# ltiao/bore

Measured on AMD Instinct MI355X. Metric: BO-iterations/sec (fit+argmax), 16-16-1 MLP, higher is better.
Workload: dtype f32; 1 GPU; BASELINE config 4 (= config 1 x independent loops): Branin-2D, 16-16-1 MLP, q=0.25, 200 epochs, batch 64, 3 L-BFGS-B restarts from 1024 samples; loops_per_gpu=512, total_loops=512, schedule=async, N_start=15, N_end=217, parallelism=replica-shard x1

## Files before the change

bore_amd/csrc/bore_argmax.hip:

```cpp
#include <hip/hip_runtime.h>

#include <cmath>
#include <cstdlib>
#include <cstring>

#include "host_common.h"
#include "lbfgsb.h"
#include "mlp_device.h"
#include "mlp_regs.h"
#include "mlp_point.h"
#include "arg_bf16_mfma.h"

using namespace bore;

__device__ __forceinline__ void labels_body(const double *y, int N, double vi, float *z,
                                            double *tau_out, const int *ids, const int *its,
                                            int n_init, long long cap, double gamma,
                                            long long model, int it_now = -1) {
  extern __shared__ float smem[];
  double *ys = reinterpret_cast<double *>(smem);
  long long stride = N;
  if (ids) {
    N = n_init + (it_now >= 0 ? it_now : uniform_i32(its[model]));
    model = uniform_i64(ids[model]);
// ... 293 lines not shown
__global__ __launch_bounds__(BORE_THREADS) void screen_topk_kernel(const ScreenArgs a) {
  screen_body<SHAPE, BF16, MODE>(a, blockIdx.x);
}

struct SampleSpec {
  uint64_t seed;
  int64_t model_index0, draw_index;
  const double *low, *high;
};

struct ScreenRequest {
  const bore_mlp_desc *desc; int n_models; const float *theta; const double *X_init; const SampleSpec *spec;
  int64_t n_samples; int x_shared, num_starts; double *x0; int32_t *idx; float *pred;
};

struct AcqKnobs { long long coop_grid = 1LL << 22, queue = -1; int waves = -1, big = -1, occ2 = -1, screen_split = -1; };
static AcqKnobs acq_knobs() {
  auto env = [](const char *name, long long unset) { return getenv(name) ? atoll(getenv(name)) : unset; };
  return AcqKnobs{env("BORE_LBFGSB_COOP_GRID", 1LL << 22), env("BORE_LBFGSB_QUEUE", -1), (int)env("BORE_LBFGSB_WAVES", -1),
                  (int)env("BORE_LBFGSB_BIG", -1), (int)env("BORE_LBFGSB_OCC2", -1), (int)env("BORE_SCREEN_SPLIT", -1)};
}

struct ScreenPlan {
  ScreenArgs a;
  size_t lds_floats;
  int flavour, parts;
};

static int screen_plan(const bore_mlp_desc *desc, int n_models, int64_t n_samples, int num_starts, bool pred,
                       const AcqKnobs &knobs, int cus, bool batch, ScreenPlan &p) {
  ScreenArgs &a = p.a;
  if (n_samples < 1 || n_samples > (1 << 20)) return fail(BORE_E_INVALID, "screen_topk: n_samples out of range");
  if (num_starts < 1 || num_starts > n_samples) return fail(BORE_E_INVALID, "screen_topk: need 1 <= num_starts <= n_samples");
  int n_pad = 1;
  while (n_pad < n_samples) n_pad <<= 1;
// ... 129 lines not shown
  (void)hipMemcpyToSymbol(HIP_SYMBOL(lbfgsb::g_lb_pp), zz, sizeof(zz));
  return (int)hipMemcpyToSymbol(HIP_SYMBOL(lbfgsb::g_lb_phase), z, sizeof(z));
}
extern "C" int bore_debug_lpp(unsigned long long *out) {
  return (int)hipMemcpyFromSymbol(out, HIP_SYMBOL(lbfgsb::g_lb_pp),
                                  sizeof(unsigned long long) * LB_PP_MAX * 64);
}
#define BORE_LCLOCK() clock64()
#else
#define BORE_LCLOCK() 0LL
#endif

#define BORE_POINT_SHAPE(S) ((S) != 1)


template <int SHAPE, bool BF16 = false, bool LEAN = false, bool ALWAYS_COOP = false, bool MAYQ = true, int PUBLISH = 0>
__device__ __forceinline__ void lbfgsb_body(const LbfgsbArgs &a, const long long model,
                                            const int block_y, const int it_now = -1) {
  extern __shared__ float smem[];
  constexpr MlpLayout Lc = bore_static_layout(SHAPE > 0 ? SHAPE : 0, 2, BORE_BATCH_MAX);
  const long long c_enter = BORE_LCLOCK();
  const MlpLayout &L = begin_kernel<SHAPE>(Lc, a.L, smem, a.total, a.o_layout);
  const long long c_begun = BORE_LCLOCK();
  int tid = threadIdx.x;
  BORE_OPAQUE_TID(tid);
  const int wv = __builtin_amdgcn_readfirstlane(tid >> 6), lane = tid & 63;
  const long long lid = a.ids ? uniform_i64(a.ids[model]) : model;
  const int n_lay = layer_count<SHAPE>(L), D = (bore_shape_takes_fewer_inputs(SHAPE) && !BF16) ? a.d_in : L.w[0];
  const int p0 = block_y * a.PB;
  const int np = min(a.PB, a.R - p0);
  float *th = smem, *tile = smem + a.o_tile, *vals = smem + a.o_vals;
  double *blo = reinterpret_cast<double *>(smem + a.o_box), *bhi = blo + D;
  int *bnbd = reinterpret_cast<int *>(bhi + D);
// ... 24 lines not shown
    while (__hip_atomic_exchange(a.big_locks + sl, 1, __ATOMIC_ACQUIRE, __HIP_MEMORY_SCOPE_AGENT) != 0)
      sl = sl + 1 == BORE_BIG_SLOTS ? 0 : sl + 1;
    qnext[1] = sl;
    qnext[2] = 0;
  }
  const int myrow = coop ? wv * 16 : wv * 16 + lane;
  const lbfgsb::Coop cp = (ALWAYS_COOP || coop) ? lbfgsb::Coop{lane, 64} : lbfgsb::Coop{0, 1};
  __syncthreads();
  double *my_big = nullptr;
  int big_slot = 0;
  if (use_big) {
    big_slot = uniform_i32(qnext[1]);
    my_big = a.big + ((size_t)big_slot * 8 + wv) * (size_t)a.big_wave;
  }
  const long long c_staged = BORE_LCLOCK();
  if (wv >= np) {
    if (use_big && lane == 0 && atomicAdd(qnext + 2, 1) == NW - 1)
      __hip_atomic_store(a.big_locks + big_slot, 0, __ATOMIC_RELEASE, __HIP_MEMORY_SCOPE_AGENT);
    return;
  }
  double *res = reinterpret_cast<double *>(smem + a.o_res);
  int *cnt = reinterpret_cast<int *>(res + (multi ? np : 4) * (D + 3));
  for (int pass = 0; pass < passes; ++pass) {
  int myp;
  if (queue) {
    int nxt = wv;
    if (pass > 0) {
      if (lane == 0) nxt = atomicAdd(qnext, 1);
      nxt = __builtin_amdgcn_readfirstlane(nxt);
    }
    myp = nxt < np ? nxt : -1;
  } else {
    myp = coop ? (wv + 4 * pass < np ? wv + 4 * pass : -1)
               : ((lane < 16 && lane * 4 + wv < np) ? lane * 4 + wv : -1);
// ... 130 lines not shown
          if constexpr (LEAN) {
            net.load_fwd(thw);
            net.template load_bwd<Net::n, 1>(thw);
          }
          static_assert(Net::KC0 == 1, "two inputs: one k-chunk");
          float xin[Net::KC0];
          xin[0] = q4 == 0 ? (float)x0 : (q4 == 1 ? (float)x1 : 0.f);
          __builtin_amdgcn_sched_barrier(0);
          const float Tv = net.fg(thw, xin, a.transform, a.sign);
          s.f = (double)__uint_as_float(__builtin_amdgcn_readfirstlane(__float_as_uint(Tv)));
          g0 = (double)__uint_as_float(__builtin_amdgcn_readfirstlane(__float_as_uint(net.d[0][0][0])));
          g1 = (double)__uint_as_float(__builtin_amdgcn_readfirstlane(__float_as_uint(net.d[0][0][1])));
          t_fg += BORE_LCLOCK() - c1;
          ++n_rounds;
        };
        lbfgsb::lbfgsb_advance<SHAPE != 1>(st, wk, blo, bhi, bnbd, a.opt, cp, evaluate, evaluate2);
      } else {
        lbfgsb::lbfgsb_advance<SHAPE != 1>(st, wk, blo, bhi, bnbd, a.opt, cp, evaluate);
      }
      t_adv = BORE_LCLOCK() - c0 - t_fg;
      done = true;
    }
  }
  if constexpr (ALWAYS_COOP) {
  } else {
  for (int round = 0; !direct && round < a.max_rounds; ++round) {
    int pending = 0;
    const long long c0 = BORE_LCLOCK();
    if (!done) {
      const int rc = lbfgsb::lbfgsb_advance<SHAPE != 1>(st, wk, blo, bhi, bnbd, a.opt, cp);
      if (rc == lbfgsb::LB_NEED_FG) {
// ... 156 lines not shown
    for (int d = 0; d < D; ++d) put(d, best >= 0 ? res[best * (D + 3) + 3 + d] : 0.0);
    put(D, (double)best);
    put(D + 1, nfev_sum);
    put(D + 2, nfev_max);
    if (a.stamps) {
      const long long *s = a.stamps + lid * 4;
      const long long now = wall_clock64();
      put(D + 3, (double)(s[1] - s[0]));
      put(D + 4, (double)(s[2] - s[1]));
      put(D + 5, (double)(s[3] - s[2]));
      put(D + 6, (double)(now - s[3]));
    } else {
      for (int i = 3; i < 7; ++i) put(D + i, 0.0);
    }
    put(D + 7, exec_sum);
    if constexpr (PUBLISH == 1) {
      asm volatile("s_waitcnt vmcnt(0)" ::: "memory");
      if (a.flag_by_store) {
        __threadfence_system();
        __hip_atomic_store(a.flag + lid, it_done + 1, __ATOMIC_RELEASE, __HIP_MEMORY_SCOPE_SYSTEM);
      } else {
        (void)__hip_atomic_exchange(a.flag + lid, it_done + 1, __ATOMIC_RELAXED, __HIP_MEMORY_SCOPE_SYSTEM);
      }
    } else {
      __threadfence_system();
      __hip_atomic_store(a.flag + lid, it_done + 1, __ATOMIC_RELEASE, __HIP_MEMORY_SCOPE_SYSTEM);
    }
  }
  }
  if (use_big) {
    asm volatile("s_waitcnt vmcnt(0)" ::: "memory");
    if (lane == 0 && atomicAdd(qnext + 2, 1) == NW - 1)
      __hip_atomic_store(a.big_locks + big_slot, 0, __ATOMIC_RELEASE, __HIP_MEMORY_SCOPE_AGENT);
  }
}

template <int SHAPE, bool BF16 = false>
__global__ __launch_bounds__(BORE_THREADS) void lbfgsb_kernel(const LbfgsbArgs a) {
  lbfgsb_body<SHAPE, BF16>(a, blockIdx.x, blockIdx.y);
}

template <int SHAPE, bool BF16 = false>
__global__ __launch_bounds__(BORE_THREADS, 2) void lbfgsb_kernel_occ2(const LbfgsbArgs a) {
// ... 399 lines not shown
```

bore_amd/csrc/bore_engine.hip:

```cpp
#include <hip/hip_runtime.h>

#include <chrono>
#include <cmath>
#include <cstdint>
#include <cstdlib>
#include <cstring>
#include <atomic>
#include <initializer_list>
#include <mutex>
#include <new>
#include <thread>
#include <vector>

#include <sched.h>

#include "../../include/bore_hip.h"
#include "host_common.h"
#include "mlp_shapes.h"

namespace {

struct Mt19937 {
  uint32_t key[624];
  int pos;
// ... 354 lines not shown
int async_create(bore_engine *e, const double *X0, const double *y0) {
  const size_t L = e->cfg.n_loops, D = e->D, R = e->cfg.num_starts, n0 = e->cfg.n_init;
  if (R > 16) return fail(BORE_E_UNSUPPORTED, "engine_create: async_loops needs num_starts <= 16");
  e->as = new (std::nothrow) Async();
  if (!e->as) return fail(BORE_E_HIP, "engine_create: out of memory");
  Async &A = *e->as;
  int rc;
  if ((rc = async_alloc(e, n0 * 2 > 128 ? n0 * 2 : 128))) return rc;
  {
    const bore_engine_cfg &c = e->cfg;
    IterEngine &E = A.eng;
    E.desc = &e->desc; E.theta = e->theta; E.adam_m = e->adam_m; E.adam_v = e->adam_v; E.adam_t = e->adam_t;
    E.gamma = c.gamma; E.epochs = c.epochs; E.batch_size = c.batch_size; E.seed = c.seed; E.loop_id0 = c.loop_id0;
    E.adam = &c.adam; E.num_samples = c.num_samples; E.low = e->low.data(); E.high = e->high.data();
    E.num_starts = c.num_starts; E.transform = c.transform; E.opts = &c.lbfgsb; E.n_loops = c.n_loops;
  }
  std::vector<float> x32(L * n0 * D);
  for (size_t i = 0; i < x32.size(); ++i) x32[i] = (float)X0[i];
  HIP_TRY(hipMemcpy2D(A.eng.X_seen, A.cap * D * 8, X0, n0 * D * 8, n0 * D * 8, L, hipMemcpyHostToDevice));
  HIP_TRY(hipMemcpy2D(A.eng.y_seen, A.cap * 8, y0, n0 * 8, n0 * 8, L, hipMemcpyHostToDevice));
  HIP_TRY(hipMemcpy2D(A.eng.X32, A.cap * D * 4, x32.data(), n0 * D * 4, n0 * D * 4, L, hipMemcpyHostToDevice));
  if ((rc = pin_alloc(&A.result, L * (D + 8))) || (rc = pin_alloc(&A.flag, L)) ||
      (rc = dev_alloc(&A.stamps, L * 4)))
    return rc;
  std::memset(A.flag, 0, L * 4);
  HIP_TRY(hipMemset(A.stamps, 0, L * 4 * 8));
  {
    int dev = 0, khz = 0;
    HIP_TRY(hipGetDevice(&dev));
    if (hipDeviceGetAttribute(&khz, hipDeviceAttributeWallClockRate, dev) == hipSuccess && khz > 0)
// ... 766 lines not shown
```

bore_amd/csrc/bore_iter.hip:

```cpp

struct QueueEntry {
  int lid, it;
};

struct IterArgs {
  FitArgs f;
  ScreenArgs s;
  LbfgsbArgs b;
  double *X_seen, *y_seen;
  float *X32, *z;
  const double *x_new, *y_new;
  long long *stamps;
  double gamma;
  int D;
  const int *targets;
  const double *ynew;
  const int *yseq;
  int *parked;
  const int *abort_flag;
  long long wait_ticks;
  const QueueEntry *q_ring;
  unsigned long long *q_head;
  int q_mask;
  const unsigned long long *q_tail_host;
// ... 3 lines not shown
__device__ __forceinline__ double load_host_f64(const double *p) {
  const long long v = __hip_atomic_load(reinterpret_cast<const long long *>(p), __ATOMIC_RELAXED,
                                        __HIP_MEMORY_SCOPE_SYSTEM);
  return __longlong_as_double(v);
}

#define BORE_LAG_YIELD_Q 3
__device__ __forceinline__ void phase_handoff() {
  __builtin_amdgcn_fence(__ATOMIC_RELEASE, "workgroup");
  asm volatile("s_waitcnt vmcnt(0) lgkmcnt(0)" ::: "memory");
  __syncthreads();
  __builtin_amdgcn_fence(__ATOMIC_ACQUIRE, "workgroup");
  asm volatile("buffer_inv sc0\n\ts_waitcnt vmcnt(0)" ::: "memory");
}

template <int SHAPE, bool LOCAL = false>
__device__ __forceinline__ void iteration_once(const IterArgs *__restrict__ pa,
                                                         const long long slot, const int it,
                                                         const bool staged, const long long t_begin = 0) {
  const IterArgs &a = *pa;
  const long long lid = uniform_i64(a.f.ids[slot]), cap = a.f.cap;
  long long *stp = a.stamps ? a.stamps + lid * 4 : nullptr;
  if (stp && threadIdx.x == 0) stp[0] = t_begin ? t_begin : wall_clock64();
  if (it > 0) {
    const long long row = a.f.n_init + it - 1;
    for (int d = threadIdx.x; d < a.D; d += blockDim.x) {
      const double v = staged ? a.x_new[slot * a.D + d] : load_host_f64(a.ynew + lid * (a.D + 1) + d);
      a.X_seen[(lid * cap + row) * a.D + d] = v;
      a.X32[(lid * cap + row) * a.D + d] = (float)v;
    }
    if (threadIdx.x == 0)
// ... 13 lines not shown
  }
  fit_body<SHAPE>(a.f, slot, it);
  if (stp && threadIdx.x == 0) stp[2] = wall_clock64();
  if constexpr (LOCAL) phase_handoff();
  else {
    __threadfence();
    __syncthreads();
  }
  screen_body<SHAPE, false>(a.s, slot, it);
  if (stp && threadIdx.x == 0) stp[3] = wall_clock64();
  if constexpr (LOCAL) phase_handoff();
  else {
    __threadfence();
    __syncthreads();
  }
  lbfgsb_body<SHAPE, false, true, true, false, LOCAL ? 1 : 0>(a.b, slot, 0, it);
}

template <int SHAPE, bool RESIDENT, int OCC = 2>
__global__ __launch_bounds__(BORE_THREADS, OCC) void iteration_kernel(const IterArgs *__restrict__ pa) {
  const long long slot = blockIdx.x;
  const int it_first = uniform_i32(pa->f.its[slot]);
  if constexpr (!RESIDENT) {
    typedef const __attribute__((address_space(4))) IterArgs *IterArgsConst1;
    const IterArgs &a = *(const IterArgs *)(IterArgsConst1) reinterpret_cast<unsigned long long>(pa);
    const long long lid = uniform_i64(a.f.ids[slot]), cap = a.f.cap;
    const int it = it_first;
    long long *stp = a.stamps ? a.stamps + lid * 4 : nullptr;
    if (stp && threadIdx.x == 0) stp[0] = wall_clock64();
    if (it > 0) {
      const long long row = a.f.n_init + it - 1;
      for (int d = threadIdx.x; d < a.D; d += blockDim.x) {
        const double v = a.x_new[slot * a.D + d];
        a.X_seen[(lid * cap + row) * a.D + d] = v;
// ... 3 lines not shown
    }
    __threadfence();
    __syncthreads();
    labels_body(a.y_seen, 0, 0.0, a.z, nullptr, a.f.ids, a.f.its, a.f.n_init, cap, a.gamma, slot);
    if (stp && threadIdx.x == 0) stp[1] = wall_clock64();
    __threadfence();
    __syncthreads();
    fit_body<SHAPE>(a.f, slot);
    if (stp && threadIdx.x == 0) stp[2] = wall_clock64();
    __threadfence();
    __syncthreads();
    screen_body<SHAPE, false>(a.s, slot);
    if (stp && threadIdx.x == 0) stp[3] = wall_clock64();
    __threadfence();
    __syncthreads();
    lbfgsb_body<SHAPE, false, true, true, false>(a.b, slot, 0);
    if (a.targets && threadIdx.x == 0 && it + 1 < a.targets[slot])
      __hip_atomic_store(a.parked + lid, it + 1, __ATOMIC_RELEASE, __HIP_MEMORY_SCOPE_SYSTEM);
    return;
  }
  __shared__ __attribute__((aligned(16))) int s_go4[4];
  const int target = pa->targets ? uniform_i32(pa->targets[slot]) : it_first + 1;
  int *prog;
  {
    unsigned long long pb = reinterpret_cast<unsigned long long>(pa) + offsetof(IterArgs, progress);
    asm volatile("" : "+s"(pb));
    prog = reinterpret_cast<int *>(pb);
  }
  for (int it = it_first;;) {
    {
      const int total = __hip_atomic_load(prog, __ATOMIC_RELAXED, __HIP_MEMORY_SCOPE_AGENT);
      const int n_wg = (int)gridDim.x;
      const int lead = uniform_i32((it - it_first) * n_wg - total);
      if (lead < -(n_wg >> 1)) __builtin_amdgcn_s_setprio(3);
      else if (lead > (n_wg >> 1)) __builtin_amdgcn_s_setprio(0);
      else __builtin_amdgcn_s_setprio(1);
    }
    unsigned long long pa_bits = reinterpret_cast<unsigned long long>(pa);
    asm volatile("" : "+s"(pa_bits));
    typedef const __attribute__((address_space(4))) IterArgs *IterArgsConst;
    iteration_once<SHAPE, true>((const IterArgs *)(IterArgsConst)pa_bits, slot, it, it == it_first);
    __syncthreads();
    ++it;
    if (threadIdx.x == 0) __hip_atomic_fetch_add(prog, 1, __ATOMIC_RELAXED, __HIP_MEMORY_SCOPE_AGENT);
    if (it >= target) break;
    if (threadIdx.x == 0) {
      const long long lid = pa->f.ids[slot], wait_ticks = pa->wait_ticks;
      const int *yseq = pa->yseq + lid, *abort_flag = pa->abort_flag;
      int go = 0;
      const long long t0 = wall_clock64();
      for (;;) {
        if (__hip_atomic_load(yseq, __ATOMIC_RELAXED, __HIP_MEMORY_SCOPE_SYSTEM) >= it) {
          asm volatile("" ::: "memory");
          go = 1;
          break;
        }
// ... 14 lines not shown
      s_go4[0] = go;
    }
    __syncthreads();
    const int go = uniform_i32(s_go4[0]);
    __syncthreads();
    if (!go) break;
  }
}

#ifdef BORE_QUEUE_STAMP_DRAW
__device__ long long g_wg_start[4096][2];
extern "C" int bore_debug_wg_starts(long long *out) {
  return (int)hipMemcpyFromSymbol(out, HIP_SYMBOL(g_wg_start), sizeof(long long) * 4096 * 2);
}
#endif
template <int SHAPE, int OCC = 2>
__global__ __launch_bounds__(BORE_THREADS, OCC) void queue_kernel(const IterArgs *__restrict__ pa) {
  __shared__ __attribute__((aligned(16))) int s_q4[4];
#ifdef BORE_QUEUE_STAMP_DRAW
  if (threadIdx.x == 0 && blockIdx.x < 4096) {
    g_wg_start[blockIdx.x][0] = wall_clock64();
    const unsigned hw = __builtin_amdgcn_s_getreg((4) | (0 << 6) | (31 << 11));
    const unsigned xcc = __builtin_amdgcn_s_getreg((20) | (0 << 6) | (31 << 11));
    g_wg_start[blockIdx.x][1] = ((long long)xcc << 32) | hw;
  }
#endif
  for (;;) {
    if (threadIdx.x == 0) {
#ifdef BORE_QUEUE_STAMP_DRAW
      const long long t_draw = wall_clock64();
      s_q4[2] = (int)(t_draw & 0xffffffffll);
// ... 33 lines not shown
      s_q4[0] = lid;
      s_q4[1] = it;
    }
    __syncthreads();
    const int lid = uniform_i32(s_q4[0]), it = uniform_i32(s_q4[1]);
#ifdef BORE_QUEUE_STAMP_DRAW
    const long long t_begin = ((long long)s_q4[3] << 32) | (unsigned)s_q4[2];
#else
    const long long t_begin = 0;
#endif
    __syncthreads();
    if (lid < 0) break;
    unsigned long long pa_bits = reinterpret_cast<unsigned long long>(pa);
    asm volatile("" : "+s"(pa_bits));
    typedef const __attribute__((address_space(4))) IterArgs *IterArgsConst;
    iteration_once<SHAPE>((const IterArgs *)(IterArgsConst)pa_bits, (long long)lid, it, false, t_begin);
    __syncthreads();
  }
}

static int iteration_shape(const bore_mlp_desc *desc) {
  if (desc->compute != BORE_COMPUTE_F32) return 0;
  const int f = bore_kernel_flavour(desc, true);
  if (f == 1) return 1;
  if (f == 5 && desc->input_dim == 16 && bore_flavour_on(5)) return 5;
  return 0;
}

static constexpr bool fused_flavour_on(int shape) { return shape == 1 || bore_flavour_on(shape); }
static constexpr int fused_most_per_cu(int shape) { return shape == 5 ? 2 : 3; }

// ... 28 lines not shown
  const bore_mlp_desc *desc;
  float *theta, *adam_m, *adam_v;
  int64_t *adam_t;
  double *X_seen, *y_seen;
  float *X32, *z;
  double gamma;
  int epochs, batch_size;
  uint64_t seed;
  int64_t loop_id0;
  const bore_adam_cfg *adam;
  int64_t num_samples;
  const double *low, *high;
  int num_starts, transform;
  const bore_lbfgsb_opts *opts;
  int n_loops;
};

struct Worker {
  hipStream_t stream = nullptr;
  hipEvent_t done = nullptr, ev[4] = {nullptr, nullptr, nullptr, nullptr};
  bool busy = false;
  int32_t *h_int = nullptr, *d_int = nullptr;
  double *h_dbl = nullptr, *d_dbl = nullptr;
  double *x0 = nullptr, *x = nullptr, *jac = nullptr, *fun = nullptr;
  int32_t *idx = nullptr, *info = nullptr;
  IterArgs *h_args = nullptr, *d_args = nullptr;
  size_t stage_bytes = 0;
};

struct IterQueue {
  const QueueEntry *ring;
  unsigned long long *head;
  int mask;
  const unsigned long long *tail_host;
  int wgs;
};

struct IterPlan {
  int shape;
  size_t lds_bytes;
  size_t part_bytes[4];
};

static int iteration_plan(const IterEngine &E, const Worker &w, int n_slots, IterArgs *h, IterPlan *plan) {
  if (!g_batch) return fail(BORE_E_INVALID, "iteration_launch: no batch set");
  const int64_t cap = g_batch->cap;
  FitPlan fit;
  ScreenPlan screen;
  LbfgsbPlan restarts;
  int rc = fit_build(FitRequest{E.desc, n_slots, E.theta, E.adam_m, E.adam_v, E.adam_t, E.X32, E.z, cap, E.epochs,
                                E.batch_size, nullptr, E.seed, E.loop_id0, 0, E.adam, nullptr},
                     fit);
  if (rc) return rc < 0 ? rc : fail(BORE_E_INVALID, "iteration_launch: epochs must be positive");
  h->f = fit.a;
  const size_t lf = fit.lds_floats;
  const int sf = fit.flavour;
// ... 15 lines not shown
  h->targets = g_batch->targets;
  h->ynew = g_batch->ynew; h->yseq = g_batch->yseq; h->parked = g_batch->parked;
  h->abort_flag = g_batch->abort_flag;
  const bool resident = g_batch->targets && g_batch->ynew && g_batch->yseq && g_batch->parked &&
                        g_batch->abort_flag;
  if (!resident) h->targets = nullptr;
  h->wait_ticks = resident ? g_batch->wait_ticks : 0;
  h->gamma = E.gamma;
  h->D = E.desc->input_dim;
  h->progress = 0;
  h->q_ring = nullptr; h->q_head = nullptr; h->q_mask = 0; h->q_tail_host = nullptr;
  size_t floats = lf > ls ? lf : ls;
  floats = floats > lb ? floats : lb;
  const size_t labels_floats = 2 * ((size_t)cap + 2);
  floats = floats > labels_floats ? floats : labels_floats;
  *plan = IterPlan{shape, floats * 4, {lf * 4, ls * 4, lb * 4, labels_floats * 4}};
  return bore_with_flavour<fused_flavour_on>(FusedFlavours{}, shape, [&](auto S) {
    int rc = 0;
    if ((rc = allow_lds(iteration_kernel<S(), true, 2>, floats * 4)) || (rc = allow_lds(iteration_kernel<S(), false, 2>, floats * 4)) ||
        (rc = allow_lds(queue_kernel<S(), 2>, floats * 4)))
      return rc;
    if constexpr (fused_most_per_cu(S()) == 3)
      if ((rc = allow_lds(iteration_kernel<S(), true, 3>, floats * 4)) || (rc = allow_lds(queue_kernel<S(), 3>, floats * 4))) return rc;
    return 0;
  });
}

template <typename K>
static int fused_launch(K kernel, int workgroups, const IterPlan &p, const Worker &w) {
  hipLaunchKernelGGL(kernel, dim3(workgroups), dim3(BORE_THREADS), p.lds_bytes, w.stream, (const IterArgs *)w.d_args);
  HIP_TRY(hipGetLastError());
  return 0;
}

static int iteration_launch_queue(const IterEngine &E, Worker &w, int n_slots, const IterQueue &q) {
  IterArgs *h = w.h_args;
  IterPlan p;
  if (const int rc = iteration_plan(E, w, n_slots, h, &p)) return rc;
  if (q.wgs < 1 || !q.ring || !q.head || !q.tail_host || !g_batch->ynew || !g_batch->abort_flag)
    return fail(BORE_E_INVALID, "iteration_launch: incomplete work queue");
  h->q_ring = q.ring; h->q_head = q.head; h->q_mask = q.mask; h->q_tail_host = q.tail_host;
  h->targets = nullptr;
  h->wait_ticks = 0;
  HIP_TRY(hipMemcpyAsync(w.d_args, h, sizeof(IterArgs), hipMemcpyHostToDevice, w.stream));
  return bore_with_flavour<fused_flavour_on>(FusedFlavours{}, p.shape, [&](auto S) {
    if constexpr (fused_most_per_cu(S()) == 3)
      if (q.wgs > 2 * device_cus()) return fused_launch(queue_kernel<S(), 3>, q.wgs, p, w);
    return fused_launch(queue_kernel<S(), 2>, q.wgs, p, w);
  });
}

static int iteration_launch(const IterEngine &E, Worker &w, int n_slots) {
  IterArgs *h = w.h_args;
  IterPlan p;
  int rc;
  if ((rc = iteration_plan(E, w, n_slots, h, &p))) return rc;
  if (h->wait_ticks > 0) {
    int per_cu = 0;
    if ((rc = iteration_loops_per_cu(p.shape, p.lds_bytes, &per_cu))) return rc;
    if (getenv("BORE_ASYNC_DEBUG"))
      fprintf(stderr, "[bore] fused kernel: %zu B of LDS per loop (fit %zu, screen %zu, restarts %zu, labels %zu), %d loops per CU\n",
              p.lds_bytes, p.part_bytes[0], p.part_bytes[1], p.part_bytes[2], p.part_bytes[3], per_cu);
    if (g_batch->resident_loops > per_cu * device_cus()) h->wait_ticks = 0;
  }
  HIP_TRY(hipMemcpyAsync(w.d_args, h, w.stage_bytes, hipMemcpyHostToDevice, w.stream));
  return bore_with_flavour<fused_flavour_on>(FusedFlavours{}, p.shape, [&](auto S) {
    if constexpr (fused_most_per_cu(S()) == 3)
      if (h->wait_ticks > 0 && g_batch->resident_loops > 2 * device_cus()) return fused_launch(iteration_kernel<S(), true, 3>, n_slots, p, w);
    if (h->wait_ticks > 0) return fused_launch(iteration_kernel<S(), true, 2>, n_slots, p, w);
    return fused_launch(iteration_kernel<S(), false, 2>, n_slots, p, w);
  });
}
```

bore_amd/csrc/lbfgsb.h:

```cpp
#pragma once
#include <math.h>
#include <stdint.h>

#include <type_traits>

#if defined(__HIPCC__)
#define LB_HD __host__ __device__ __forceinline__
#define LB_HDN __host__ __device__ __forceinline__
#else
#define LB_HD inline
#define LB_HDN
#endif

namespace lbfgsb {

enum { LB_NEED_FG = 1, LB_DONE = 2 };

enum {
  T_START = 0, T_NEW_X = 1, T_FG = 3, T_CONVERGENCE = 4, T_STOP = 5, T_ERROR = 7, T_ABNORMAL = 8
};
enum {
  M_NONE = 0, M_PGTOL = 401, M_FACTR = 402, M_MAXFUN = 502, M_MAXITER = 504,
  M_NO_FEASIBLE = 701, M_FACTR_NEG = 702, M_M_LE_0 = 711, M_N_LE_0 = 712, M_INVALID_NBD = 713
};
// ... 1567 lines not shown
    if (nbd[i] == 2 || nbd[i] == 3) xi = fmin(xi, u[i]);
    w.x[i] = xi;
    w.g[i] = 0.0;
  }
  s.f = 0.0;
  s.stage = S_INIT;
  s.task = T_START;
  s.msg = M_NONE;
  s.nit = 0;
  s.nfev = 0;
  s.status = 2;
}

struct ReverseCommunication {};
struct NoTwoVariableForm {};
template <bool VL = true, class FG = ReverseCommunication, class FG2 = NoTwoVariableForm>
LB_HD int lbfgsb_advance(State &s, const Work &w, const double *l, const double *u,
                         const int *nbd, const Options &opt, const Coop coop_in = Coop{0, 1},
                         FG fg = FG{}, FG2 fg2 = FG2{}) {
  constexpr bool DIRECT = !std::is_same<FG, ReverseCommunication>::value;
  constexpr bool TWO = DIRECT && !std::is_same<FG2, NoTwoVariableForm>::value;
  Coop coop = coop_in;
  const int n = LB_UNI(s.n, coop_in), m = LB_UNI(s.m, coop_in);
  bool first_ls = false;
  bool resume_ls = (s.stage == S_FG_LNSRCH);

  if (s.stage == S_FINISHED) return LB_DONE;
  bool big_stale = w.vm == LB_BIG_LAZY;
  if (!DIRECT && big_stale && s.stage == S_INIT) zero_big(w, m, coop_in);
  LB_MARK(s, 15);

  auto save_evaluated_point = [&]() {
    LB_PHASE_BEGIN(20);
    for (int i = coop.lane; i < n; i += coop.nl) { w.xlast[i] = w.x[i]; w.glast[i] = w.g[i]; }
    LB_LANES_SYNC();
    s.flast = s.f;
// ... 112 lines not shown
      s.ginit = s.gtest = s.gx = s.gy = s.finit = s.fx = s.fy = s.stx = s.sty = s.stmin = s.stmax = 0.0;
      s.width = s.width1 = 0.0;
      s.xstep = s.gd = s.gdold = s.stp = s.dtd = s.dnorm = s.stpmx = s.fold = 0.0;
      s.ifun = s.iback = 0;
      s.iword = -1;
      if (!s.cnstnd && s.col > 0) {
        LB_EVENT(s, EV_UNCONSTRAINED_ITERATION);
        for (int i = coop.lane; i < n; i += coop.nl) w.z[i] = w.x[i];
        LB_LANES_SYNC();
        s.wrk = s.updatd;
        s.nseg = 0;
      } else {
        const IterArgs ia{n, m, LB_UNI(s.col, coop), LB_UNI(s.head, coop), LB_UNI(s.nfree, coop),
                          LB_UNI(s.nenter, coop), LB_UNI(s.ileave, coop), LB_UNI(s.updatd, coop),
                          LB_UNI(s.iupdat, coop), s.theta, s.sbgnrm, coop};
        LB_PHASE_BEGIN(21);
        const int rc = cauchy<VL>(ia, w, l, u, nbd);
        LB_PHASE_END(0);
        s.nseg = rc >> 8;
        if (rc & 0xff) {
          LB_EVENT(s, EV_CAUCHY_SINGULAR_REFRESH);
          refresh_memory(s);
          continue;
        }
        {
          LB_PHASE_BEGIN(22);
          freev<VL>(s, w, coop);
          LB_PHASE_END(8);
        }
        if (s.nenter > 0) LB_EVENT(s, EV_ENTER);
        if (s.ileave < n + 1) LB_EVENT(s, EV_LEAVE);
        s.nact = n - s.nfree;
      }
      if (s.nfree == 0) LB_EVENT(s, EV_NFREE_ZERO);
      if (s.nfree != 0 && s.col != 0) {
        const IterArgs ia{n, m, LB_UNI(s.col, coop), LB_UNI(s.head, coop), LB_UNI(s.nfree, coop),
                          LB_UNI(s.nenter, coop), LB_UNI(s.ileave, coop), LB_UNI(s.updatd, coop),
                          LB_UNI(s.iupdat, coop), s.theta, s.sbgnrm, coop};
        if (s.wrk) {
          LB_PHASE_BEGIN(23);
          if (DIRECT && big_stale) {
            zero_big(w, m, coop);
            big_stale = false;
          }
          const int fk = formk(ia, w);
          LB_PHASE_END(1);
          if (fk) { LB_EVENT(s, EV_FORMK_REFRESH); refresh_memory(s); continue; }
        }
        int rc;
        {
          LB_PHASE_BEGIN(24);
          const int cm = cmprlb(s, w, coop);
          LB_PHASE_END(2);
          if (cm) { LB_EVENT(s, EV_CMPRLB_REFRESH); refresh_memory(s); continue; }
        }
        {
          LB_PHASE_BEGIN(25);
          rc = subsm<VL>(ia, w, l, u, nbd);
          LB_PHASE_END(3);
        }
        s.iword = rc >> 8;
        if (rc & 0xff) { LB_EVENT(s, EV_SUBSM_REFRESH); refresh_memory(s); continue; }
        if (s.iword == 1) LB_EVENT(s, EV_SUBSM_HIT_BOUND);
      }
      {
        LB_PHASE_BEGIN(26);
        for (int i = coop.lane; i < n; i += coop.nl) w.d[i] = w.z[i] - w.x[i];
        LB_LANES_SYNC();
        LB_PHASE_END(12);
      }
      first_ls = true;
    }

    s.info = 0;
    int ls_rc;
    {
      LB_PHASE_BEGIN(27);
      ls_rc = lnsrlb<VL>(s, w, l, u, nbd, first_ls ? 1 : 0, coop);
// ... 183 lines not shown
```

Baseline: 291,000 BO-iterations/s.

## Offload L-BFGS-B formk to idle helper waves via an LDS job board

Adds a workgroup-local job board so that waves left idle (when there are 4 or fewer restarts per block) can compute formk for active restarts. The restart wave posts its formk job and runs cmprlb meanwhile. It also posts a speculative formk before the Cauchy step, double-buffering the big matrix so the speculative result can be committed if no variables enter or leave. This aims to hide formk latency on the critical path, at the cost of atomic handshakes, spin-waiting, extra LDS for the spare buffers, and extra kernel instantiations. It is enabled by default for shape 1.

```diff
diff --git a/bore_amd/csrc/bore_argmax.hip b/bore_amd/csrc/bore_argmax.hip
--- a/bore_amd/csrc/bore_argmax.hip
+++ b/bore_amd/csrc/bore_argmax.hip
@@ -331,11 +331,17 @@
   int64_t n_samples; int x_shared, num_starts; double *x0; int32_t *idx; float *pred;
 };
 
-struct AcqKnobs { long long coop_grid = 1LL << 22, queue = -1; int waves = -1, big = -1, occ2 = -1, screen_split = -1; };
+#define BORE_HELPER_DEFAULT 1
+struct AcqKnobs {
+  long long coop_grid = 1LL << 22, queue = -1; int waves = -1, big = -1, occ2 = -1, screen_split = -1;
+  int helper = BORE_HELPER_DEFAULT;
+};
 static AcqKnobs acq_knobs() {
   auto env = [](const char *name, long long unset) { return getenv(name) ? atoll(getenv(name)) : unset; };
+  const int helper = (int)env("BORE_LBFGSB_HELPER", BORE_HELPER_DEFAULT);
   return AcqKnobs{env("BORE_LBFGSB_COOP_GRID", 1LL << 22), env("BORE_LBFGSB_QUEUE", -1), (int)env("BORE_LBFGSB_WAVES", -1),
-                  (int)env("BORE_LBFGSB_BIG", -1), (int)env("BORE_LBFGSB_OCC2", -1), (int)env("BORE_SCREEN_SPLIT", -1)};
+                  (int)env("BORE_LBFGSB_BIG", -1), (int)env("BORE_LBFGSB_OCC2", -1), (int)env("BORE_SCREEN_SPLIT", -1),
+                  helper >= 0 && helper <= 3 ? helper : BORE_HELPER_DEFAULT};
 }
 
 struct ScreenPlan {
@@ -495,9 +501,114 @@
 #define BORE_POINT_SHAPE(S) ((S) != 1)
 
 
-template <int SHAPE, bool BF16 = false, bool LEAN = false, bool ALWAYS_COOP = false, bool MAYQ = true, int PUBLISH = 0>
+enum { JOB_FREE = 0, JOB_POSTED = 1, JOB_TAKEN = 2, JOB_DONE = 3, JOB_WITHDRAWN = 4, JOB_INTS = 16 };
+enum { JOBS_SPECULATIVE = 0, JOBS_COMMITTED, JOBS_DROPPED, JOBS_TAKEN, JOBS_WITHDRAWN, JOBS_COUNTERS };
+__device__ unsigned long long g_helper_stats[JOBS_COUNTERS];
+extern "C" int bore_debug_helper_stats(long long *out, int reset) {
+  static const unsigned long long zero[JOBS_COUNTERS] = {0};
+  if (out) HIP_TRY(hipMemcpyFromSymbol(out, HIP_SYMBOL(g_helper_stats), sizeof(zero)));
+  if (reset) HIP_TRY(hipMemcpyToSymbol(HIP_SYMBOL(g_helper_stats), zero, sizeof(zero)));
+  return 0;
+}
+struct RestartJobs {
+  int *slot;
+  int *stats;
+  lbfgsb::Work *wk;
+  double *blk0, *blk1;
+  double *rwn0, *rwn1;
+  int lane, mode;
+  int live = 0;
+  int pending = 0;
+  int guess_nfree = 0;
+  int how = 0;
+  __device__ __forceinline__ void count(int which) const {
+    if (lane == 0) __hip_atomic_fetch_add(stats + which, 1, __ATOMIC_RELAXED, __HIP_MEMORY_SCOPE_WORKGROUP);
+  }
+  __device__ __forceinline__ void put(const lbfgsb::IterArgs &ia, int speculative) const {
+    if (lane == 0) {
+      slot[2] = ia.col; slot[3] = ia.head; slot[4] = ia.nfree; slot[5] = ia.nenter; slot[6] = ia.ileave;
+      slot[7] = ia.updatd; slot[8] = ia.iupdat; slot[9] = speculative; slot[10] = live;
+      *reinterpret_cast<double *>(slot + 12) = ia.theta;
+      __hip_atomic_store(slot, (int)JOB_POSTED, __ATOMIC_RELEASE, __HIP_MEMORY_SCOPE_WORKGROUP);
+    }
+  }
+  __device__ __forceinline__ bool withdraw() const {
+    int ok = 0;
+    if (lane == 0) {
+      int seen = JOB_POSTED;
+      ok = __hip_atomic_compare_exchange_strong(slot, &seen, (int)JOB_WITHDRAWN, __ATOMIC_ACQ_REL, __ATOMIC_ACQUIRE,
+                                                __HIP_MEMORY_SCOPE_WORKGROUP) ? 1 : 0;
+    }
+    return __builtin_amdgcn_readfirstlane(ok) != 0;
+  }
+  __device__ __forceinline__ int wait_done() const {
+    while (__builtin_amdgcn_readfirstlane(__hip_atomic_load(slot, __ATOMIC_ACQUIRE, __HIP_MEMORY_SCOPE_WORKGROUP)) != JOB_DONE)
+      __builtin_amdgcn_s_sleep(1);
+    return __builtin_amdgcn_readfirstlane(slot[1]);
+  }
+  __device__ __forceinline__ void speculate(const lbfgsb::IterArgs &guess, const lbfgsb::Work &) {
+    if (!mode || !blk1) return;
+    put(guess, 1);
+    pending = 1;
+    guess_nfree = guess.nfree;
+    count(JOBS_SPECULATIVE);
+  }
+  __device__ __forceinline__ void drop() {
+    if (!pending) return;
+    if (!withdraw()) (void)wait_done();
+    pending = 0;
+    count(JOBS_DROPPED);
+  }
+  __device__ __forceinline__ void post(const lbfgsb::IterArgs &ia, const lbfgsb::Work &) {
+    if (!mode) return;
+    how = 0;
+    if (pending) {
+      if (mode != 2 && ia.nenter == 0 && ia.ileave == ia.n + 1 && ia.nfree == guess_nfree) {
+        how = 1;
+        return;
+      }
+      if (!withdraw()) {
+        how = 2;
+        return;
+      }
+      pending = 0;
+      count(JOBS_DROPPED);
+    }
+    put(ia, 0);
+  }
+  __device__ __forceinline__ int collect(const lbfgsb::IterArgs &ia, const lbfgsb::Work &w) {
+    if (!mode) return lbfgsb::formk(ia, w);
+    if (how == 2) {
+      (void)wait_done();
+      pending = 0;
+      count(JOBS_DROPPED);
+      return lbfgsb::formk(ia, w);
+    }
+    if (withdraw()) {
+      pending = 0;
+      count(JOBS_WITHDRAWN);
+      return lbfgsb::formk(ia, w);
+    }
+    const int rc = wait_done();
+    if (how == 1) {
+      live ^= 1;
+      wk->snd = live ? blk1 : blk0;
+      wk->wn = wk->snd + 2 * ia.m;
+      wk->rwn = live ? rwn1 : rwn0;
+      pending = 0;
+      count(JOBS_COMMITTED);
+    } else {
+      count(JOBS_TAKEN);
+    }
+    return rc;
+  }
+};
+
+template <int SHAPE, bool BF16 = false, bool LEAN = false, bool ALWAYS_COOP = false, bool MAYQ = true, int PUBLISH = 0,
+          bool HELPER = false>
 __device__ __forceinline__ void lbfgsb_body(const LbfgsbArgs &a, const long long model,
                                             const int block_y, const int it_now = -1) {
+  static_assert(!HELPER || (SHAPE == 1 && !BF16 && ALWAYS_COOP && !MAYQ), "the job board: the fused float32 kernels of shape 1");
   extern __shared__ float smem[];
   constexpr MlpLayout Lc = bore_static_layout(SHAPE > 0 ? SHAPE : 0, 2, BORE_BATCH_MAX);
   const long long c_enter = BORE_LCLOCK();
@@ -552,10 +663,17 @@
     my_big = a.big + ((size_t)big_slot * 8 + wv) * (size_t)a.big_wave;
   }
   const long long c_staged = BORE_LCLOCK();
+  const bool helping = HELPER && np <= 4 && a.queue != 0;
+  int *const job_slots = reinterpret_cast<int *>(vals);
+  double *const spares = HELPER && a.big_wave > 0 ? reinterpret_cast<double *>(smem + a.big_wave) : nullptr;
   if (wv >= np) {
+    if constexpr (HELPER) {
+      if (!helping) return;
+    } else {
     if (use_big && lane == 0 && atomicAdd(qnext + 2, 1) == NW - 1)
       __hip_atomic_store(a.big_locks + big_slot, 0, __ATOMIC_RELEASE, __HIP_MEMORY_SCOPE_AGENT);
     return;
+    }
   }
   double *res = reinterpret_cast<double *>(smem + a.o_res);
   int *cnt = reinterpret_cast<int *>(res + (multi ? np : 4) * (D + 3));
@@ -716,7 +834,16 @@
           t_fg += BORE_LCLOCK() - c1;
           ++n_rounds;
         };
+        if constexpr (HELPER) {
+          const int nb = lbfgsb::big_size(a.opt.m);
+          double *const spare = spares ? spares + (size_t)myp * (nb + 2 * a.opt.m) : nullptr;
+          const RestartJobs jobs{job_slots + myp * JOB_INTS, execs + 4, &wk, wk.snd, spare, wk.rwn,
+                                 spare ? spare + nb : nullptr, lane, helping ? a.queue : 0};
+          lbfgsb::lbfgsb_advance<SHAPE != 1>(st, wk, blo, bhi, bnbd, a.opt, cp, evaluate, evaluate2, jobs);
+          if (helping && lane == 0) __hip_atomic_fetch_add(qnext, 1, __ATOMIC_RELEASE, __HIP_MEMORY_SCOPE_WORKGROUP);
+        } else {
         lbfgsb::lbfgsb_advance<SHAPE != 1>(st, wk, blo, bhi, bnbd, a.opt, cp, evaluate, evaluate2);
+        }
       } else {
         lbfgsb::lbfgsb_advance<SHAPE != 1>(st, wk, blo, bhi, bnbd, a.opt, cp, evaluate);
       }
@@ -903,6 +1030,11 @@
       for (int i = 3; i < 7; ++i) put(D + i, 0.0);
     }
     put(D + 7, exec_sum);
+    if constexpr (HELPER) {
+      for (int c = 0; c < JOBS_COUNTERS; ++c)
+        if (const int v = execs[4 + c])
+          __hip_atomic_fetch_add(g_helper_stats + c, (unsigned long long)v, __ATOMIC_RELAXED, __HIP_MEMORY_SCOPE_AGENT);
+    }
     if constexpr (PUBLISH == 1) {
       asm volatile("s_waitcnt vmcnt(0)" ::: "memory");
       if (a.flag_by_store) {
@@ -916,6 +1048,59 @@
       __hip_atomic_store(a.flag + lid, it_done + 1, __ATOMIC_RELEASE, __HIP_MEMORY_SCOPE_SYSTEM);
     }
   }
+  }
+  if constexpr (HELPER) {
+    const bool take = a.queue != 3;
+    while (helping) {
+      int took = -1;
+      if (lane == 0 && take)
+        for (int j = 0; j < np; ++j) {
+          int *sl = job_slots + j * JOB_INTS;
+          if (__hip_atomic_load(sl, __ATOMIC_RELAXED, __HIP_MEMORY_SCOPE_WORKGROUP) != JOB_POSTED) continue;
+          int seen = JOB_POSTED;
+          if (__hip_atomic_compare_exchange_strong(sl, &seen, (int)JOB_TAKEN, __ATOMIC_ACQUIRE, __ATOMIC_RELAXED,
+                                                   __HIP_MEMORY_SCOPE_WORKGROUP)) {
+            took = j;
+            break;
+          }
+        }
+      took = __builtin_amdgcn_readfirstlane(took);
+      if (took >= 0) {
+        int *sl = job_slots + took * JOB_INTS;
+        float *base = smem + a.o_prob + (size_t)took * a.prob_floats;
+        lbfgsb::Work w = lbfgsb::make_work(reinterpret_cast<double *>(base + a.o_dw),
+                                           reinterpret_cast<int *>(base + a.o_iw), D, a.opt.m, nullptr);
+        __builtin_amdgcn_fence(__ATOMIC_ACQUIRE, "workgroup");
+        {
+          const int speculative = uniform_i32(sl[9]), live = uniform_i32(sl[10]), nb = lbfgsb::big_size(a.opt.m);
+          double *b0 = w.snd, *b1 = spares ? spares + (size_t)took * (nb + 2 * a.opt.m) : b0;
+          double *src = live ? b1 : b0, *dst = speculative ? (live ? b0 : b1) : src;
+          if (dst != b0) w.rwn = b1 + nb;
+          if (speculative) {
+            for (int i = 2 * lane; i < nb; i += 128) {
+              const double v0 = src[i], v1 = src[i + 1];
+              dst[i] = v0;
+              dst[i + 1] = v1;
+            }
+            wave_lds_sync();
+          }
+          w.snd = dst;
+          w.wn = dst + 2 * a.opt.m;
+        }
+        const lbfgsb::IterArgs ia{D, a.opt.m, uniform_i32(sl[2]), uniform_i32(sl[3]), uniform_i32(sl[4]),
+                                  uniform_i32(sl[5]), uniform_i32(sl[6]), uniform_i32(sl[7]), uniform_i32(sl[8]),
+                                  *reinterpret_cast<const double *>(sl + 12), 0.0, lbfgsb::Coop{lane, 64}};
+        const int rc = lbfgsb::formk(ia, w);
+        wave_lds_sync();
+        if (lane == 0) {
+          sl[1] = rc;
+          __hip_atomic_store(sl, (int)JOB_DONE, __ATOMIC_RELEASE, __HIP_MEMORY_SCOPE_WORKGROUP);
+        }
+        continue;
+      }
+      if (uniform_i32(__hip_atomic_load(qnext, __ATOMIC_RELAXED, __HIP_MEMORY_SCOPE_WORKGROUP)) >= np) break;
+      __builtin_amdgcn_s_sleep(4);
+    }
   }
   if (use_big) {
     asm volatile("s_waitcnt vmcnt(0)" ::: "memory");
diff --git a/bore_amd/csrc/bore_engine.hip b/bore_amd/csrc/bore_engine.hip
--- a/bore_amd/csrc/bore_engine.hip
+++ b/bore_amd/csrc/bore_engine.hip
@@ -392,6 +392,7 @@
     E.gamma = c.gamma; E.epochs = c.epochs; E.batch_size = c.batch_size; E.seed = c.seed; E.loop_id0 = c.loop_id0;
     E.adam = &c.adam; E.num_samples = c.num_samples; E.low = e->low.data(); E.high = e->high.data();
     E.num_starts = c.num_starts; E.transform = c.transform; E.opts = &c.lbfgsb; E.n_loops = c.n_loops;
+    E.helper = acq_knobs().helper;
   }
   std::vector<float> x32(L * n0 * D);
   for (size_t i = 0; i < x32.size(); ++i) x32[i] = (float)X0[i];
diff --git a/bore_amd/csrc/bore_iter.hip b/bore_amd/csrc/bore_iter.hip
--- a/bore_amd/csrc/bore_iter.hip
+++ b/bore_amd/csrc/bore_iter.hip
@@ -41,7 +41,7 @@
   asm volatile("buffer_inv sc0\n\ts_waitcnt vmcnt(0)" ::: "memory");
 }
 
-template <int SHAPE, bool LOCAL = false>
+template <int SHAPE, bool LOCAL = false, bool HELPER = false>
 __device__ __forceinline__ void iteration_once(const IterArgs *__restrict__ pa,
                                                          const long long slot, const int it,
                                                          const bool staged, const long long t_begin = 0) {
@@ -85,10 +85,10 @@
     __threadfence();
     __syncthreads();
   }
-  lbfgsb_body<SHAPE, false, true, true, false, LOCAL ? 1 : 0>(a.b, slot, 0, it);
-}
-
-template <int SHAPE, bool RESIDENT, int OCC = 2>
+  lbfgsb_body<SHAPE, false, true, true, false, LOCAL ? 1 : 0, HELPER>(a.b, slot, 0, it);
+}
+
+template <int SHAPE, bool RESIDENT, int OCC = 2, bool HELPER = false>
 __global__ __launch_bounds__(BORE_THREADS, OCC) void iteration_kernel(const IterArgs *__restrict__ pa) {
   const long long slot = blockIdx.x;
   const int it_first = uniform_i32(pa->f.its[slot]);
@@ -122,7 +122,7 @@
     if (stp && threadIdx.x == 0) stp[3] = wall_clock64();
     __threadfence();
     __syncthreads();
-    lbfgsb_body<SHAPE, false, true, true, false>(a.b, slot, 0);
+    lbfgsb_body<SHAPE, false, true, true, false, 0, HELPER>(a.b, slot, 0);
     if (a.targets && threadIdx.x == 0 && it + 1 < a.targets[slot])
       __hip_atomic_store(a.parked + lid, it + 1, __ATOMIC_RELEASE, __HIP_MEMORY_SCOPE_SYSTEM);
     return;
@@ -147,7 +147,7 @@
     unsigned long long pa_bits = reinterpret_cast<unsigned long long>(pa);
     asm volatile("" : "+s"(pa_bits));
     typedef const __attribute__((address_space(4))) IterArgs *IterArgsConst;
-    iteration_once<SHAPE, true>((const IterArgs *)(IterArgsConst)pa_bits, slot, it, it == it_first);
+    iteration_once<SHAPE, true, HELPER>((const IterArgs *)(IterArgsConst)pa_bits, slot, it, it == it_first);
     __syncthreads();
     ++it;
     if (threadIdx.x == 0) __hip_atomic_fetch_add(prog, 1, __ATOMIC_RELAXED, __HIP_MEMORY_SCOPE_AGENT);
@@ -192,7 +192,7 @@
   return (int)hipMemcpyFromSymbol(out, HIP_SYMBOL(g_wg_start), sizeof(long long) * 4096 * 2);
 }
 #endif
-template <int SHAPE, int OCC = 2>
+template <int SHAPE, int OCC = 2, bool HELPER = false>
 __global__ __launch_bounds__(BORE_THREADS, OCC) void queue_kernel(const IterArgs *__restrict__ pa) {
   __shared__ __attribute__((aligned(16))) int s_q4[4];
 #ifdef BORE_QUEUE_STAMP_DRAW
@@ -256,7 +256,7 @@
     unsigned long long pa_bits = reinterpret_cast<unsigned long long>(pa);
     asm volatile("" : "+s"(pa_bits));
     typedef const __attribute__((address_space(4))) IterArgs *IterArgsConst;
-    iteration_once<SHAPE>((const IterArgs *)(IterArgsConst)pa_bits, (long long)lid, it, false, t_begin);
+    iteration_once<SHAPE, false, HELPER>((const IterArgs *)(IterArgsConst)pa_bits, (long long)lid, it, false, t_begin);
     __syncthreads();
   }
 }
@@ -315,6 +315,7 @@
   int num_starts, transform;
   const bore_lbfgsb_opts *opts;
   int n_loops;
+  int helper;
 };
 
 struct Worker {
@@ -341,6 +342,7 @@
   int shape;
   size_t lds_bytes;
   size_t part_bytes[4];
+  int helper;
 };
 
 static int iteration_plan(const IterEngine &E, const Worker &w, int n_slots, IterArgs *h, IterPlan *plan) {
@@ -386,9 +388,19 @@
   floats = floats > lb ? floats : lb;
   const size_t labels_floats = 2 * ((size_t)cap + 2);
   floats = floats > labels_floats ? floats : labels_floats;
-  *plan = IterPlan{shape, floats * 4, {lf * 4, ls * 4, lb * 4, labels_floats * 4}};
+  const int helper = shape == 1 && E.num_starts <= 4 ? E.helper : 0;
+  h->b.queue = helper;
+  if (helper) {
+    const size_t at = (lb + 3) & ~(size_t)3, need = 2 * ((size_t)lbfgsb::big_size(E.opts->maxcor) + 2 * (size_t)E.opts->maxcor) * E.num_starts;
+    h->b.big_wave = at + need <= floats ? (int)at : 0;
+  }
+  *plan = IterPlan{shape, floats * 4, {lf * 4, ls * 4, lb * 4, labels_floats * 4}, helper};
   return bore_with_flavour<fused_flavour_on>(FusedFlavours{}, shape, [&](auto S) {
     int rc = 0;
+    if constexpr (S() == 1)
+      if ((rc = allow_lds(iteration_kernel<1, true, 2, true>, floats * 4)) || (rc = allow_lds(iteration_kernel<1, false, 2, true>, floats * 4)) ||
+          (rc = allow_lds(queue_kernel<1, 2, true>, floats * 4)))
+        return rc;
     if ((rc = allow_lds(iteration_kernel<S(), true, 2>, floats * 4)) || (rc = allow_lds(iteration_kernel<S(), false, 2>, floats * 4)) ||
         (rc = allow_lds(queue_kernel<S(), 2>, floats * 4)))
       return rc;
@@ -403,6 +415,12 @@
   hipLaunchKernelGGL(kernel, dim3(workgroups), dim3(BORE_THREADS), p.lds_bytes, w.stream, (const IterArgs *)w.d_args);
   HIP_TRY(hipGetLastError());
   return 0;
+}
+
+static void fused_without_board(IterArgs *h, IterPlan &p) {
+  p.helper = 0;
+  h->b.queue = 0;
+  h->b.big_wave = 0;
 }
 
 static int iteration_launch_queue(const IterEngine &E, Worker &w, int n_slots, const IterQueue &q) {
@@ -414,10 +432,13 @@
   h->q_ring = q.ring; h->q_head = q.head; h->q_mask = q.mask; h->q_tail_host = q.tail_host;
   h->targets = nullptr;
   h->wait_ticks = 0;
+  if (fused_most_per_cu(p.shape) == 3 && q.wgs > 2 * device_cus()) fused_without_board(h, p);
   HIP_TRY(hipMemcpyAsync(w.d_args, h, sizeof(IterArgs), hipMemcpyHostToDevice, w.stream));
   return bore_with_flavour<fused_flavour_on>(FusedFlavours{}, p.shape, [&](auto S) {
     if constexpr (fused_most_per_cu(S()) == 3)
       if (q.wgs > 2 * device_cus()) return fused_launch(queue_kernel<S(), 3>, q.wgs, p, w);
+    if constexpr (S() == 1)
+      if (p.helper) return fused_launch(queue_kernel<1, 2, true>, q.wgs, p, w);
     return fused_launch(queue_kernel<S(), 2>, q.wgs, p, w);
   });
 }
@@ -435,10 +456,16 @@
               p.lds_bytes, p.part_bytes[0], p.part_bytes[1], p.part_bytes[2], p.part_bytes[3], per_cu);
     if (g_batch->resident_loops > per_cu * device_cus()) h->wait_ticks = 0;
   }
+  if (fused_most_per_cu(p.shape) == 3 && h->wait_ticks > 0 && g_batch->resident_loops > 2 * device_cus()) fused_without_board(h, p);
   HIP_TRY(hipMemcpyAsync(w.d_args, h, w.stage_bytes, hipMemcpyHostToDevice, w.stream));
   return bore_with_flavour<fused_flavour_on>(FusedFlavours{}, p.shape, [&](auto S) {
     if constexpr (fused_most_per_cu(S()) == 3)
       if (h->wait_ticks > 0 && g_batch->resident_loops > 2 * device_cus()) return fused_launch(iteration_kernel<S(), true, 3>, n_slots, p, w);
+    if constexpr (S() == 1)
+      if (p.helper) {
+        if (h->wait_ticks > 0) return fused_launch(iteration_kernel<1, true, 2, true>, n_slots, p, w);
+        return fused_launch(iteration_kernel<1, false, 2, true>, n_slots, p, w);
+      }
     if (h->wait_ticks > 0) return fused_launch(iteration_kernel<S(), true, 2>, n_slots, p, w);
     return fused_launch(iteration_kernel<S(), false, 2>, n_slots, p, w);
   });
diff --git a/bore_amd/csrc/lbfgsb.h b/bore_amd/csrc/lbfgsb.h
--- a/bore_amd/csrc/lbfgsb.h
+++ b/bore_amd/csrc/lbfgsb.h
@@ -1605,12 +1605,15 @@
 
 struct ReverseCommunication {};
 struct NoTwoVariableForm {};
-template <bool VL = true, class FG = ReverseCommunication, class FG2 = NoTwoVariableForm>
+struct NoJobBoard {};
+template <bool VL = true, class FG = ReverseCommunication, class FG2 = NoTwoVariableForm, class JB = NoJobBoard>
 LB_HD int lbfgsb_advance(State &s, const Work &w, const double *l, const double *u,
                          const int *nbd, const Options &opt, const Coop coop_in = Coop{0, 1},
-                         FG fg = FG{}, FG2 fg2 = FG2{}) {
+                         FG fg = FG{}, FG2 fg2 = FG2{}, JB jobs = JB{}) {
   constexpr bool DIRECT = !std::is_same<FG, ReverseCommunication>::value;
   constexpr bool TWO = DIRECT && !std::is_same<FG2, NoTwoVariableForm>::value;
+  constexpr bool JOBS = DIRECT && !std::is_same<JB, NoJobBoard>::value;
+  (void)jobs;
   Coop coop = coop_in;
   const int n = LB_UNI(s.n, coop_in), m = LB_UNI(s.m, coop_in);
   bool first_ls = false;
@@ -1753,12 +1756,21 @@
         const IterArgs ia{n, m, LB_UNI(s.col, coop), LB_UNI(s.head, coop), LB_UNI(s.nfree, coop),
                           LB_UNI(s.nenter, coop), LB_UNI(s.ileave, coop), LB_UNI(s.updatd, coop),
                           LB_UNI(s.iupdat, coop), s.theta, s.sbgnrm, coop};
+        if constexpr (JOBS) {
+          if (ia.updatd && ia.col > 0 && ia.nfree > 0) {
+            IterArgs guess = ia;
+            guess.nenter = 0;
+            guess.ileave = n + 1;
+            jobs.speculate(guess, w);
+          }
+        }
         LB_PHASE_BEGIN(21);
         const int rc = cauchy<VL>(ia, w, l, u, nbd);
         LB_PHASE_END(0);
         s.nseg = rc >> 8;
         if (rc & 0xff) {
           LB_EVENT(s, EV_CAUCHY_SINGULAR_REFRESH);
+          if constexpr (JOBS) jobs.drop();
           refresh_memory(s);
           continue;
         }
@@ -1776,7 +1788,30 @@
         const IterArgs ia{n, m, LB_UNI(s.col, coop), LB_UNI(s.head, coop), LB_UNI(s.nfree, coop),
                           LB_UNI(s.nenter, coop), LB_UNI(s.ileave, coop), LB_UNI(s.updatd, coop),
                           LB_UNI(s.iupdat, coop), s.theta, s.sbgnrm, coop};
-        if (s.wrk) {
+        if constexpr (JOBS) {
+          const bool wrk = s.wrk != 0;
+          if (wrk) {
+            LB_PHASE_BEGIN(23);
+            if (big_stale) {
+              zero_big(w, m, coop);
+              big_stale = false;
+            }
+            jobs.post(ia, w);
+            LB_PHASE_END(1);
+          } else {
+            jobs.drop();
+          }
+          LB_PHASE_BEGIN(24);
+          const int cm = cmprlb(s, w, coop);
+          LB_PHASE_END(2);
+          if (wrk) {
+            LB_PHASE_BEGIN(23);
+            const int fk = jobs.collect(ia, w);
+            LB_PHASE_END(1);
+            if (fk) { LB_EVENT(s, EV_FORMK_REFRESH); refresh_memory(s); continue; }
+          }
+          if (cm) { LB_EVENT(s, EV_CMPRLB_REFRESH); refresh_memory(s); continue; }
+        } else if (s.wrk) {
           LB_PHASE_BEGIN(23);
           if (DIRECT && big_stale) {
             zero_big(w, m, coop);
@@ -1787,7 +1822,7 @@
           if (fk) { LB_EVENT(s, EV_FORMK_REFRESH); refresh_memory(s); continue; }
         }
         int rc;
-        {
+        if constexpr (!JOBS) {
           LB_PHASE_BEGIN(24);
           const int cm = cmprlb(s, w, coop);
           LB_PHASE_END(2);
@@ -1801,6 +1836,8 @@
         s.iword = rc >> 8;
         if (rc & 0xff) { LB_EVENT(s, EV_SUBSM_REFRESH); refresh_memory(s); continue; }
         if (s.iword == 1) LB_EVENT(s, EV_SUBSM_HIT_BOUND);
+      } else {
+        if constexpr (JOBS) jobs.drop();
       }
       {
         LB_PHASE_BEGIN(26);
```

Result: faster. 296,600 BO-iterations/s, median of 6 (+1.9%).
